# kngwyu/rogue-gym

Measured on AMD Instinct MI355X. Metric: env-steps/sec (whole node) at 65 536 envs, 32x16 mini-dungeon, higher is better.
Workload: dtype u8/u16 integer state, f32 observation; 1 GPU; config-mini.json 32x16, 65536 envs per GPU (65536 total), gray-image obs [N,1,16,32] f32, max_steps 1000, auto-reset; envs_per_gpu=65536, parallelism=env-sharded x1, no data-path collective

## Files before the change

### __graft_entry__.py

```python
import os
import subprocess
import sys

ROOT = os.path.dirname(os.path.abspath(__file__))
PKG = os.path.join(ROOT, "rogue-gym_amd")
for p in (ROOT, PKG):
    if p not in sys.path:
        sys.path.insert(0, p)


def source_id():
    import hashlib
    csrc = os.path.join(PKG, "csrc")
    files = sorted(os.path.join(csrc, f) for f in os.listdir(csrc) if f.endswith((".hip", ".cpp", ".h"))) + [os.path.join(ROOT, "include", "rogue_gym_hip.h")]
    h = hashlib.sha256()
    for f in files:
        h.update(os.path.basename(f).encode() + b"\0")
        h.update(open(f, "rb").read())
    return h.hexdigest()[:16]


def library_id(so):
    if not os.path.exists(so):
        return None
    blob = open(so, "rb").read()
    i = blob.find(b"RGBUILDID:")
    return blob[i + 10:i + 26].decode("ascii", "replace") if i >= 0 else None


def build():
    csrc = os.path.join(PKG, "csrc")
    so = os.path.join(PKG, "librogue_gym_hip.so")
    hipcc = "hipcc" if subprocess.call(["which", "hipcc"], stdout=subprocess.DEVNULL) == 0 else "/opt/rocm/bin/hipcc"
    sid = source_id()
    dev_so = os.path.join(PKG, "variants", "librogue_gym_hip_dev.so")
    nov_so = os.path.join(PKG, "librogue_gym_novelty.so")
    if library_id(so) != sid or library_id(dev_so) != sid or library_id(nov_so) != sid:
        have_hipcc = subprocess.call(["which", hipcc], stdout=subprocess.DEVNULL, stderr=subprocess.DEVNULL) == 0 or os.path.exists(hipcc)
        if have_hipcc:
            bdir = os.path.join(PKG, "build")
            os.makedirs(bdir, exist_ok=True)
            os.makedirs(os.path.dirname(dev_so), exist_ok=True)
            flags = ["--offload-arch=gfx950", "-std=c++17", "-fPIC", "-Wall", "-Wno-unused-function", '-DRG_BUILD_ID="%s"' % sid]
            objs, dev_objs, jobs = [], [], []
            for src, opt, has_knobs in (("rg_kernels.hip", "-O3", True), ("rg_regen_lanes.hip", "-O3", True), ("rg_obs.hip", "-Os", True), ("rg_crop_typed.hip", "-Os", False), ("rg_pixels.hip", "-Os", False), ("rg_action_mask.hip", "-Os", False), ("rg_path.hip", "-O3", False), ("rg_route.hip", "-O3", False), ("rg_episode.hip", "-O3", False), ("rg_monsters.hip", "-O3", False), ("rg_objects.hip", "-O3", False), ("rg_state_io.hip", "-O3", False), ("rg_api.cpp", "-O2", True), ("rg_config.cpp", "-O2", False),
                                        ("rg_items.cpp", "-O2", False)):
                obj = os.path.join(bdir, src.rsplit(".", 1)[0] + ".o")
                jobs.append(subprocess.Popen([hipcc] + flags + [opt, "-c", os.path.join(csrc, src), "-o", obj]))
                objs.append(obj)
                if has_knobs:
                    dobj = os.path.join(bdir, src.rsplit(".", 1)[0] + ".dev.o")
                    jobs.append(subprocess.Popen([hipcc] + flags + ["-DRG_DEV_KNOBS", opt, "-c", os.path.join(csrc, src), "-o", dobj]))
                    dev_objs.append(dobj)
                else:
                    dev_objs.append(obj)
            nov_obj = os.path.join(bdir, "rg_novelty.o")
            jobs.append(subprocess.Popen([hipcc] + flags + ["-O3", "-c", os.path.join(csrc, "rg_novelty.hip"), "-o", nov_obj]))
            if any(j.wait() != 0 for j in jobs):
                raise RuntimeError("hipcc failed")
            subprocess.check_call([hipcc, "--offload-arch=gfx950", "-shared", nov_obj, "-o", nov_so])
            link_nov = ["-L" + PKG, "-lrogue_gym_novelty"]
            subprocess.check_call([hipcc, "--offload-arch=gfx950", "-shared"] + objs + link_nov + ["-Wl,-rpath,$ORIGIN", "-o", so])
            subprocess.check_call([hipcc, "--offload-arch=gfx950", "-shared"] + dev_objs + link_nov + ["-Wl,-rpath,$ORIGIN/..", "-o", dev_so])
        elif not os.path.exists(so):
            raise RuntimeError("hipcc not found and librogue_gym_hip.so is not prebuilt")
        else:
            print("warning: hipcc not found; the prebuilt librogue_gym_hip.so (build id %s) does not match the sources (%s)" % (library_id(so), sid), file=sys.stderr)
    from oracle import pyoracle
    pyoracle.build()
    import rogue_gym
    from rogue_gym_python import _rogue_gym
    _rogue_gym.load_library()


def smoke():
    import json
    import numpy as np
    build()
    sys.path.insert(0, os.path.join(ROOT, "tests"))
    from parity_util import ACTION_KEYS, lockstep
    with open(os.path.join(ROOT, "tests", "golden", "reference_goldens.json")) as f:
        cfg = json.load(f)["configs"]["mini"]
    rng = np.random.RandomState(0)
    n, steps = 256, 64
    keys = [ACTION_KEYS[rng.randint(0, 11, n)] for _ in range(steps)]
    hip, _ = lockstep(cfg, list(range(n)), keys, max_steps=40, check_every=8, internal_every=32)
    obs = hip.obs(0, 0, False)
    assert obs.shape == (n, 1, 16, 32)
    print("smoke ok: %d envs x %d steps bit-exact vs oracle" % (n, steps))


if __name__ == "__main__":
    build()
    if len(sys.argv) > 1 and sys.argv[1] == "smoke":
# ... 2 lines not shown
```

### rogue-gym_amd/csrc/rg_api.cpp

```cpp
#include <hip/hip_runtime.h>
#include <dlfcn.h>

#include <algorithm>
#include <cstdio>
#include <cstdlib>
#include <cstring>
#include <mutex>
#include <random>
#include <string>
#include <vector>

#include "../../include/rogue_gym_hip.h"
#include "rg_state.h"
#include "rg_state_io.h"
#include "rg_readers_host.h"
#include "rg_pixels.h"

extern "C" {
typedef struct ncclComm *ncclComm_t;
typedef struct { char internal[128]; } ncclUniqueId;
typedef int ncclResult_t;
typedef int ncclDataType_t;
}
static const ncclResult_t ncclSuccess = 0;
static const ncclDataType_t ncclUint8 = 1;

extern "C" {
void rgk_build(const RgState *S, const RgConfig *c, hipStream_t st);
int rgk_step(const RgState *S, const RgState *SP_dev, const RgConfig *c, const uint8_t *keys, int use_spares, int parity, hipStream_t st, hipEvent_t ev0, hipEvent_t ev1);
void rgk_probe_clock(unsigned long long *out, int spin, hipStream_t st);
void rgk_regen(const RgState *SP, const RgConfig *c, int bulk, int spares, const uint32_t *mark, uint32_t target, uint32_t *err_any, hipStream_t st, hipEvent_t ev0, hipEvent_t ev1);
void rgk_regen_gate(const uint32_t *mark, uint32_t target, uint32_t *err_any, hipStream_t st);
void rgk_export(const RgState *S, uint32_t *err_any, void *o_screen, void *o_hist, void *o_status, void *o_flags, uint32_t *o_err, hipStream_t st);
int rgk_regen_lanes_supported(const RgConfig *c, int maze_cap);
int rgk_step_bound_capable(const RgConfig *c);
int rgk_regen_lanes(const RgState *SP, const RgConfig *c, uint32_t *q, int32_t *list, int bulk, int waves, int slots, hipStream_t st, hipEvent_t ev0, hipEvent_t ev1);
void rgk_debug_descend(const RgState *S, const RgConfig *c, hipStream_t st);
void rgk_render(const RgState *S, const RgConfig *c, hipStream_t st);
void rgk_encode(const uint8_t *screen, const uint8_t *hist, const int32_t *status, uint32_t *flags, uint32_t *err_any, int n, int hw, size_t rs, size_t rst,
                int symbols, int planes_sym, uint32_t sflag, int with_hist, int kind, float *out, const int32_t *ext, hipStream_t st);
void rgk_pack(const RgState *S, int with_hist, uint8_t *out, hipStream_t st);
void rgk_scatter_rows(const void *src, void *dst, const int32_t *ext, int n, int row_bytes, hipStream_t st);
void rgk_gather_keys(const uint8_t *keys, const int32_t *ext, uint8_t *dst, int n, hipStream_t st);
int rgk_obs(const RgState *S, const RgConfig *c, uint32_t sflag, int with_hist, int kind, float *out, uint32_t *err_any, int planes_sym, int bound, hipStream_t st, hipEvent_t ev0, hipEvent_t ev1);
int rgk_redraw(const RgState *S, const RgConfig *c, hipStream_t st);
int rgk_obs_tail_capable(const RgState *S, const RgConfig *c);
int rgk_step_tail_capable(const RgConfig *c);
int rgk_step_enc_helpers(int n, int want);
void rgk_obs_resid(const RgState *S, const RgConfig *c, float *out, hipStream_t st, hipEvent_t ev0, hipEvent_t ev1);
int rgk_obs_typed(const RgState *S, const RgConfig *c, int kind, int dtype, uint32_t sflag, int with_hist, int planes_sym, void *out, uint32_t *err_any, hipStream_t st, hipEvent_t ev0,
                  hipEvent_t ev1);
int rgk_crop_typed(const RgState *S, const RgConfig *c, int kind, int dtype, int ry, int rx, uint32_t sflag, int with_hist, int planes_sym, void *out, int32_t *centers,
                   uint32_t *err_any, hipStream_t st, hipEvent_t ev0, hipEvent_t ev1);
int rgk_pixels(const RgState *S, const RgConfig *c, const uint8_t *tiles, int th, int channels, int ry, int rx, uint8_t *out, int32_t *centers, hipStream_t st, hipEvent_t ev0,
               hipEvent_t ev1);
void rgk_action_mask(const RgState *S, const RgConfig *c, const uint8_t *keys, int n_keys, uint8_t *mask, uint8_t *sample, uint64_t seed, uint64_t draw, hipStream_t st,
                     hipEvent_t ev0, hipEvent_t ev1);
void rgk_path(const RgState *S, const RgConfig *c, uint32_t goals, const int32_t *gcell, uint16_t *field, int32_t *dist, uint8_t *key, hipStream_t st);
void rgk_route(const RgState *S, const RgConfig *c, uint32_t goals, uint32_t fallback, uint32_t mode, const int32_t *gcell, int32_t *dist, uint8_t *key, uint8_t *tier,
               hipStream_t st);
void rgk_episode(const RgState *S, const RgConfig *c, const RgEpisode *A, int slots, const int32_t *ids, const uint8_t *mask, int cut, int record, uint32_t serial,
                 hipStream_t st);
void rgk_novelty(const RgState *S, const RgConfig *c, const RgNovelty *A, int slots, const int32_t *ids, const uint8_t *mask, int cut, hipStream_t st);
void rgk_monsters(const RgState *S, const RgConfig *c, uint32_t mode, int cap, int16_t *table, int32_t *threat, hipStream_t st);
void rgk_objects(const RgState *S, const RgConfig *c, uint32_t kinds, uint32_t mode, int cap, int16_t *table, int32_t *count, hipStream_t st);
void rgk_state_save(const RgState *S, const RgIoLayout *L, const uint64_t *desc, const uint32_t *guard, const int32_t *ids, int k, uint8_t *out, hipStream_t st);
void rgk_state_load(const RgState *S, const RgIoLayout *L, const uint64_t *desc, const uint32_t *guard, const int32_t *ids, int k, const uint8_t *recs, uint32_t rec_bytes, uint8_t *ok,
                    uint8_t *mark, hipStream_t st);
void rgk_state_stairs(const RgState *S, const RgIoLayout *L, uint8_t *mark, hipStream_t st);
void rgk_reset_compact(const uint8_t *mask, int n, int32_t *list, uint32_t *cnt, hipStream_t st);
void rgk_build_list(const RgState *S, const RgConfig *c, const int32_t *list, const uint32_t *cnt, uint8_t *mark, hipStream_t st);
}

#define RG_ENC_DELAY_TICKS 2500u
#define RG_TIMED_KERNELS 5
struct rg_handle {
    RgParsed parsed;
    RgConfig cfg;
    RgState S;
    RgState SP;
    bool spares = false;
    uint32_t *lane_q = nullptr; int32_t *lane_list = nullptr;
    hipStream_t side3 = nullptr;
    hipStream_t side2 = nullptr;
    int lane_flip = 0;
    uint64_t lane_last = 0;
    uint8_t *pin_keys = nullptr;
    uint32_t *pin_err = nullptr;
    bool lane_regen = false;
    uint64_t step_count = 0;
    hipStream_t side = nullptr;
    int regen_idle_after = -1;
    int regen_bulk = 0;
    int device = 0;
    hipStream_t stream = nullptr;
    std::vector<void *> allocs;
    uint32_t *d_err = nullptr;
    uint8_t *d_keys = nullptr;
    bool render_pending = false;
    float *bound_out = nullptr; int bound_kind = 0; bool bound_valid = false;
    int32_t *obs_list_mem = nullptr; uint32_t *obs_cnt_mem = nullptr; float *gray_lut_mem = nullptr;
    bool tail_enc = false, tail_enc_off = false;
    int enc_helpers = 0;
    int bound_steps = 0;
    int stair_gen = 0;
    float *obs_scratch = nullptr;
    size_t obs_scratch_cap = 0;
    std::vector<uint64_t> seed_lo, seed_hi;
    std::vector<uint8_t> reseed;
    std::vector<uint64_t> range_lo, range_span;
    unsigned long long *d_probe = nullptr;
    std::vector<rg_handle *> sub;
    std::vector<int> g_of, l_of;
    int32_t *d_ext = nullptr;
    std::vector<int32_t> ext;
    uint8_t *d_keys_sub = nullptr;
    int planes_sym = 0;
    bool screens_stale = true;
    bool mixed = false;
    std::vector<size_t> ragged_off;
    size_t stat_rows = 0;
    RgState *d_SP = nullptr;
    ncclComm_t comm = nullptr;
    int comm_rank = 0, comm_world = 1;
    std::string err;
    bool timing = false;
    std::vector<hipEvent_t> ev[RG_TIMED_KERNELS];
    size_t ev_used[RG_TIMED_KERNELS] = {0, 0, 0, 0, 0};
    uint64_t timing_seq[RG_TIMED_KERNELS] = {0, 0, 0, 0, 0};
    uint64_t timing_stride = 1;
    uint64_t state_fp = 0;
    uint64_t *io_desc = nullptr;
    uint32_t *io_guard = nullptr;
    uint32_t io_words = 0;
    int32_t *io_ids = nullptr; size_t io_ids_cap = 0;
// ... 426 lines not shown
    return upload_seeds(h, (size_t)n);
}

int rg_reset(rg_t *h) {
    HIPCHK(h, hipSetDevice(h->device));
    if (!h->sub.empty()) {
        for (rg_handle *sh : h->sub) SUBCHK(h, sh, rg_reset(sh));
        h->screens_stale = true;
        return assemble_small(h);
    }
    h->S.stair_gen = h->stair_gen++;
    { TimedLaunch t(h, 3); rgk_build(&h->S, &h->cfg, h->stream); }
    HIPCHK(h, hipGetLastError());
    h->render_pending = true;
    h->bound_valid = false;
    return 0;
}

static int obs_common(rg_t *h, uint32_t status_flag, int with_hist, int kind, float *out_dev);
int rg_step(rg_t *h, const uint8_t *keys, int keys_on_device) { return rg_step_prefix(h, keys, h->S.n, keys_on_device); }
int rg_step_obs_gray(rg_t *h, const uint8_t *keys, int keys_on_device, uint32_t status_flag, int with_hist, float *out_dev) {
    const bool enc = h->tail_enc && !h->tail_enc_off && h->sub.empty() && (status_flag & 0x1ffu) == 0 && !with_hist && !h->bound_out && out_dev && rgk_obs_tail_capable(&h->S, &h->cfg);
    if (enc) {
        h->S.enc_out = out_dev;
        h->S.enc_helpers = h->enc_helpers;
    }
    const int rc = rg_step_prefix(h, keys, h->S.n, keys_on_device);
    h->S.enc_out = nullptr;
    h->S.enc_helpers = 0;
    if (rc) return 1;
    if (!enc) return obs_common(h, status_flag, with_hist, 0, out_dev);
    {
        TimedLaunch t(h, 2, true);
        rgk_obs_resid(&h->S, &h->cfg, out_dev, h->stream, t.start_ev(), t.stop_ev());
    }
    HIPCHK(h, hipGetLastError());
    h->render_pending = false;
    h->bound_valid = false;
    h->bound_steps = 0;
    return 0;
}

int rg_step_prefix(rg_t *h, const uint8_t *keys, int n_keys, int keys_on_device) {
    HIPCHK(h, hipSetDevice(h->device));
    if (n_keys < 0) { h->err = "rg_step_prefix: negative key count"; return 1; }
    if (n_keys > h->S.n) n_keys = h->S.n;
    if (!h->sub.empty()) {
        const uint8_t *dkeys = keys;
        if (!keys_on_device) {
            if (!h->d_keys && !dev_alloc(h, &h->d_keys, (size_t)h->S.n)) return 1;
            HIPCHK(h, hipMemcpyAsync(h->d_keys, keys, (size_t)n_keys, hipMemcpyHostToDevice, h->stream));
            dkeys = h->d_keys;
        }
        for (rg_handle *sh : h->sub) {
            int m = 0;
            while (m < sh->S.n && sh->ext[m] < n_keys) m++;
            if (m) rgk_gather_keys(dkeys, sh->d_ext, sh->d_keys_sub, m, h->stream);
            SUBCHK(h, sh, rg_step_prefix(sh, sh->d_keys_sub, m, 1));
        }
        HIPCHK(h, hipGetLastError());
        h->screens_stale = true;
        return assemble_small(h);
    }
    if (flush_render(h)) return 1;
    const uint8_t *dk = keys;
    if (!keys_on_device) {
        HIPCHK(h, hipMemcpyAsync(h->d_keys, keys, (size_t)n_keys, hipMemcpyHostToDevice, h->stream));
// ... 47 lines not shown
    }
    uint32_t err = 0;
    HIPCHK(h, hipMemcpyAsync(&err, h->d_err, 4, hipMemcpyDeviceToHost, h->stream));
    HIPCHK(h, hipStreamSynchronize(h->stream));
    if (h->side) { HIPCHK(h, hipStreamSynchronize(h->side)); HIPCHK(h, hipStreamSynchronize(h->side2)); HIPCHK(h, hipStreamSynchronize(h->side3)); }
    if (err) {
        HIPCHK(h, hipMemsetAsync(h->d_err, 0, 4, h->stream));
        if (err & RG_FLAG_ERR_INTERNAL) h->err = "internal capacity guard of the HIP stepper tripped (please report the config), or rg_reset_envs was given a device-side env id out of range";
        else if (err & RG_FLAG_ERR_STATE) h->err = "state record refused: it does not fit this env (magic / version / config fingerprint / geometry), the env is unchanged";
        else if (err & RG_FLAG_ERR_KEY) h->err = "Invalid input (key is not in the ai keymap)";
        else if (err & RG_FLAG_ERR_DEAD) h->err = "Ignored input (action while the player is dead)";
        else h->err = "Invalid tile in symbol image (symbol >= symbols - 1)";
        return 1;
    }
    return 0;
}

static int flush_mirrors(rg_handle *h) { return h->sub.empty() ? flush_render(h) : assemble_screens(h); }
int rg_screen(rg_t *h, uint8_t **dev) { if (refuse_mixed(h, "rg_screen")) return 1; HIPCHK(h, hipSetDevice(h->device)); if (flush_mirrors(h)) return 1; *dev = h->S.screen; return 0; }
int rg_hist(rg_t *h, uint8_t **dev) { if (refuse_mixed(h, "rg_hist")) return 1; HIPCHK(h, hipSetDevice(h->device)); if (flush_mirrors(h)) return 1; *dev = h->S.hist; return 0; }
int rg_status(rg_t *h, int32_t **dev) { *dev = h->S.status; return 0; }
int rg_flags(rg_t *h, uint32_t **dev) { HIPCHK(h, hipSetDevice(h->device)); if (flush_mirrors(h)) return 1; *dev = h->S.flags; return 0; }
int rg_reward(rg_t *h, float **dev) { *dev = h->S.reward; return 0; }
int rg_done(rg_t *h, uint8_t **dev) { *dev = h->S.done; return 0; }
int rg_set_stair_reward(rg_t *h, float bonus) {
    if (!(bonus == bonus) || bonus < 0.f) { h->err = "rg_set_stair_reward: the bonus must be a number >= 0"; return 1; }
    h->S.stair_reward = bonus;
    for (rg_handle *sh : h->sub) sh->S.stair_reward = bonus;
    return 0;
}

int rg_tail_encode(rg_t *h, int on) {
    h->tail_enc_off = on == 0;
    for (rg_handle *sh : h->sub) sh->tail_enc_off = on == 0;
    return 0;
}

int rg_obs_channels(const rg_t *h, int symbol, uint32_t status_flag, int with_hist) {
    return (symbol ? h->planes_sym : 1) + __builtin_popcount(status_flag & 0x1ffu) + (with_hist ? 1 : 0);
}

static int symbols_check(rg_t *h, const std::string &w, const rg_handle *sh) {
    if (sh->cfg.symbols <= h->planes_sym) return 0;
    h->err = w + "symbol image: a config of the batch has more symbols (" + std::to_string(sh->cfg.symbols) + ") than env 0's (" + std::to_string(h->planes_sym) +
             "), which sets the channel count (python/src/lib.rs:281-285)";
    return 1;
}
static int obs_common(rg_t *h, uint32_t status_flag, int with_hist, int kind, float *out_dev) {
    if (refuse_mixed(h, kind ? "rg_obs_symbol" : "rg_obs_gray")) return 1;
    HIPCHK(h, hipSetDevice(h->device));
    if (!h->sub.empty()) {
        for (rg_handle *sh : h->sub) {
            if (kind && symbols_check(h, "", sh)) return 1;
            SUBCHK(h, sh, obs_common(sh, status_flag, with_hist, kind, out_dev));
        }
        return 0;
    }
    {
        TimedLaunch t(h, 2, true);
        const bool bound = h->bound_out && out_dev == h->bound_out && kind == h->bound_kind && (status_flag & 0x1ffu) == 0 && !with_hist;
        if (rgk_obs(&h->S, &h->cfg, status_flag & 0x1ffu, with_hist ? 1 : 0, kind, out_dev, h->d_err, h->planes_sym, bound && h->S.obs_list && h->bound_valid && h->bound_steps == 1, h->stream, t.start_ev(), t.stop_ev())) {
            HIPCHK(h, hipGetLastError());
            h->render_pending = false;
            h->bound_valid = bound;
            h->bound_steps = 0;
            return 0;
        }
// ... 1313 lines not shown
```

### rogue-gym_amd/csrc/rg_obs.hip

```cpp
#include <cstdlib>
#include "rg_device.h"

#define RENDER_THREADS 256
__device__ __forceinline__ bool in_same_room(const RgState &S, const RgConfig &c, int e, int ax, int ay, int bx, int by) {
    int id = room_id_of(c, ax, ay);
    if (id < 0 || room_id_of(c, bx, by) != id) return false;
    uint8_t meta = S.room_meta[id * S.n + e];
    if ((meta & RM_KIND_MASK) == RK_EMPTY) return true;
    int x0, y0, x1, y1;
    unpack_rect(S.room_rect[id * S.n + e], x0, y0, x1, y1);
    bool ina = ax >= x0 && ax < x1 && ay >= y0 && ay < y1, inb = bx >= x0 && bx < x1 && by >= y0 && by < y1;
    return ina == inb;
}

__global__ void __launch_bounds__(RENDER_THREADS) k_render(RgState S, RgConfig c) {
    __shared__ uint8_t s_scr[RG_MAX_W * RG_MAX_H];
    const int tid = threadIdx.x, W = c.width, H = c.height, HW = W * H, n = S.n;
    const int nrooms = c.room_num_x * c.room_num_y;
    for (int e = blockIdx.x; e < n; e += gridDim.x) {
        const uint32_t fl = S.flags[e];
        if (!(fl & RG_FLAG_REDRAW)) continue;
        const uint16_t *cell = S.cell + (size_t)e * HW;
        const bool upd_hist = !(fl & RG_FLAG_HIST_STALE);
        uint8_t *hist = S.hist + (size_t)e * HW;
// ... 89 lines not shown
    for (size_t g = (size_t)blockIdx.x * blockDim.x + threadIdx.x; g < total; g += (size_t)gridDim.x * blockDim.x) {
        int e = (int)(g / q), i = (int)(g - (size_t)e * q);
        uint32_t s4 = reinterpret_cast<const uint32_t *>(screen + (size_t)e * rs)[i];
        uint32_t a = tile_to_sym(s4 & 0xff), b = tile_to_sym((s4 >> 8) & 0xff), cc = tile_to_sym((s4 >> 16) & 0xff), d = tile_to_sym(s4 >> 24);
        if (a >= symbol_max || b >= symbol_max || cc >= symbol_max || d >= symbol_max) {
            if (flags) atomicOr(&flags[e], RG_FLAG_ERR_TILE);
            atomicOr(err_any, RG_FLAG_ERR_TILE);
        }
        float4 *o = reinterpret_cast<float4 *>(out + (size_t)(ext ? ext[e] : e) * nplanes * hw) + i;
        for (uint32_t ch = 0; ch < (uint32_t)planes_sym; ch++) {
            float4 v;
            v.x = a == ch ? 1.f : 0.f; v.y = b == ch ? 1.f : 0.f; v.z = cc == ch ? 1.f : 0.f; v.w = d == ch ? 1.f : 0.f;
            if (ch >= symbol_max) v.x = v.y = v.z = v.w = 0.f;
            o[(size_t)ch * q] = v;
        }
        int p = planes_sym;
        for (int bb = 0; bb < 9; bb++)
            if (sflag & (1u << bb)) {
                float f = (float)status[(size_t)e * rst + kStatusIdx[bb]];
                float4 sv; sv.x = sv.y = sv.z = sv.w = f;
                o[(size_t)p * q] = sv;
                p++;
            }
        if (with_hist) {
            uint32_t h4 = reinterpret_cast<const uint32_t *>(hist + (size_t)e * rs)[i];
            float4 hv;
            hv.x = (h4 & 0xff) ? 1.f : 0.f; hv.y = (h4 & 0xff00) ? 1.f : 0.f; hv.z = (h4 & 0xff0000) ? 1.f : 0.f; hv.w = (h4 >> 24) ? 1.f : 0.f;
            o[(size_t)p * q] = hv;
        }
    }
}

#define OBS_THREADS 256
__device__ __forceinline__ void store_obs(float4 *p, float4 v) {
    typedef float f4v __attribute__((ext_vector_type(4)));
    f4v nv = {v.x, v.y, v.z, v.w};
#ifdef RG_EXP_OBS_PLAIN_STORES
    *reinterpret_cast<f4v *>(p) = nv;
#else
    __builtin_nontemporal_store(nv, reinterpret_cast<f4v *>(p));
#endif
}
struct ObsTabs { uint32_t w[RG_OBS_REC_WORDS(RG_OBS_MAX_ROOMS)]; };
#define OBS_ENV_BYTES(hw) ((((size_t)(hw) + sizeof(ObsTabs)) + 15) & ~(size_t)15)

__device__ __forceinline__ void draw_cells8(uint4 v, int i, int W, int HW, uint32_t g[2], uint32_t hb[2]) {
    const uint32_t q[4] = {v.x, v.y, v.z, v.w};
    g[0] = g[1] = hb[0] = hb[1] = 0;
#pragma unroll
    for (int t = 0; t < 8; t++) {
        uint32_t cw = (q[t >> 1] >> ((t & 1) * 16)) & 0xffff;
        int idx = i * 8 + t;
        bool inner = idx >= W && idx < HW - W;
        uint32_t gl = ' ';
        if (inner && (cw & C_VISIBLE)) gl = glyph_of(cw);
        if (inner && (cw & (C_VISIBLE | C_DRAWN))) gl = ((cw & C_GOLD) ? (uint32_t)'*' : gl) | 0x80u;
        g[t >> 2] |= gl << ((t & 3) * 8);
        hb[t >> 2] |= ((cw & C_VISITED) ? 1u : 0u) << ((t & 3) * 8);
    }
}
__device__ __forceinline__ bool monster_shown(const RgConfig &c, const ObsTabs *tb, int nrooms, int px, int py, int x, int y) {
    int dx = px - x, dy = py - y;
    bool show = dx * dx + dy * dy <= 2;
    if (!show) {
        int id = room_id_of(c, px, py);
        if (id >= 0 && room_id_of(c, x, y) == id) {
            if ((reinterpret_cast<const uint8_t *>(&tb->w[2 * nrooms + 1])[id] & RM_KIND_MASK) == RK_EMPTY) show = true;
            else {
                int x0, y0, x1, y1;
                unpack_rect(tb->w[nrooms + 1 + id], x0, y0, x1, y1);
                bool ina = px >= x0 && px < x1 && py >= y0 && py < y1, inb = x >= x0 && x < x1 && y >= y0 && y < y1;
                show = ina == inb;
            }
        }
    }
    return show;
}

template <int KIND, bool GROUPS, bool BOUND = false>
__global__ void __launch_bounds__(OBS_THREADS) k_obs(RgState S, RgConfig c, uint32_t sflag, int with_hist, float *__restrict__ out,
                                                    uint32_t *__restrict__ err_any, int tpe, int epb, int planes_sym, int hi_prio) {
    if (hi_prio) __builtin_amdgcn_s_setprio(3);
    extern __shared__ __align__(16) uint8_t smem[];
    float *lutf = reinterpret_cast<float *>(smem);
    uint8_t *luts = smem + 512;
    uint8_t *mtile = smem + 512 + 128;
    uint8_t *envs = smem + 512 + 128 + 64;
    const int tid = threadIdx.x, W = c.width, H = c.height, HW = W * H, Q8 = HW >> 3;
    const int32_t *list = BOUND ? S.obs_list + (size_t)S.obs_par * S.n : nullptr;
    const int n = BOUND ? (int)S.obs_cnt[S.obs_par] : S.n;
    const int nrooms = c.room_num_x * c.room_num_y;
    const int symbols = c.symbols;
    for (int g = tid; g < 128; g += blockDim.x) {
        uint32_t sy = tile_to_sym((uint32_t)g);
        luts[g] = (uint8_t)sy;
        lutf[g] = (float)(uint8_t)sy / (float)(uint8_t)symbols;
    }
    for (int g = tid; g < RG_MAX_ENEMY_KINDS + 6; g += blockDim.x) mtile[g] = c.mon[g].tile;
    const int le = tid / tpe, lt = tid - le * tpe;
    const int base_planes = KIND ? (GROUPS ? planes_sym : symbols) : 1;
    const int nplanes = base_planes + __popc(sflag) + (with_hist ? 1 : 0);
    uint8_t *scr = envs + (size_t)le * OBS_ENV_BYTES(HW);
    ObsTabs *tb = reinterpret_cast<ObsTabs *>(scr + HW);
    struct Pre { uint4 v0; uint32_t rec; };
    const int rec_words = RG_OBS_REC_WORDS(nrooms);
    const uint32_t *rec_all = S.obs_rec;
    const int stride = gridDim.x * epb;
    const int Q4 = HW >> 2;
    const bool one_wave = blockDim.x == WAVE;
    const bool fast_ok = (epb == 1 || one_wave) && Q4 <= 4 * tpe && sflag == 0 && !with_hist;
// ... 125 lines not shown
        if (redraw && lt == 0 && (scr[py * W + px] & 0x80u)) scr[py * W + px] = (uint8_t)(0x80u | '@');
        lds_barrier();
        if (with_hist) __syncthreads();
        if (staged) {
            uint32_t *m4 = reinterpret_cast<uint32_t *>(S.screen + (size_t)e * HW);
            const uint32_t *scr4 = reinterpret_cast<const uint32_t *>(scr);
            const uint32_t *hist4 = reinterpret_cast<const uint32_t *>(S.hist + (size_t)e * HW);
            const int xe = GROUPS ? __builtin_amdgcn_readfirstlane(S.ext[e]) : e;
            float4 *o = reinterpret_cast<float4 *>(out + (size_t)xe * nplanes * HW);
            float stf[9];
            int nst = 0;
            for (int b = 0; b < 9; b++)
                if (sflag & (1u << b)) stf[nst++] = (float)S.status[(size_t)e * 10 + kStatusIdx[b]];
            bool bad = false;
            for (int q = lt; q < Q4; q += tpe) {
                const uint32_t g = scr4[q] & 0x7f7f7f7fu;
                if (redraw) m4[q] = g;
                emit(o, q, g, stf, nst, hist4, bad);
            }
            if (KIND == 1 && bad) { atomicOr(&S.flags[e], RG_FLAG_ERR_TILE); atomicOr(err_any, RG_FLAG_ERR_TILE); }
            const uint32_t seen = BOUND ? RG_FLAG_SCR_CHANGED : 0u;
            if (redraw && lt == 0) {
                const uint32_t clr = seen | RG_FLAG_REDRAW | RG_FLAG_HIST_STALE | RG_FLAG_HIST_LAG | ((fl & RG_FLAG_HIST_STALE) ? 0u : RG_FLAG_HIST_DIRTY);
                const uint32_t set = (fl & RG_FLAG_HIST_STALE) ? RG_FLAG_HIST_LAG : 0u;
                if (KIND == 1) {
                    atomicAnd(&S.flags[e], ~clr);
                    if (set) atomicOr(&S.flags[e], set);
                } else S.flags[e] = (fl & ~clr) | set;
            } else if (BOUND && !redraw && lt == 0) atomicAnd(&S.flags[e], ~RG_FLAG_SCR_CHANGED);
        }
    }
}

#define RG_OBS_REDRAW_ENV() \
    lds_barrier();                                                                                                             \
    if (lane < rec_words) tb.w[lane] = t_rec;                                                                                                                            \
                           \
    const bool upd_hist = !(fle & RG_FLAG_HIST_STALE) && (fle & RG_FLAG_HIST_DIRTY);                                                                                     \
    if (lane < Q8) {                                                                                                                                                     \
        uint32_t g[2], hb[2];                                                                                                                                            \
        draw_cells8(v, lane, W, HW, g, hb);                                                                                                                              \
        reinterpret_cast<uint2 *>(scr)[lane] = make_uint2(g[0], g[1]);                                                                                                   \
        if (upd_hist) reinterpret_cast<uint2 *>(S.hist + (size_t)e * HW)[lane] = make_uint2(hb[0], hb[1]);                                                               \
    }                                                                                                                                                                    \
    lds_barrier();                                                                                                                                                       \
                                                                      \
    const uint32_t ppos = tb.w[nrooms];                                                                                                                                  \
    const int px = POS_X(ppos), py = POS_Y(ppos);                                                                                                                        \
    if (lane < nrooms) {                                                                                                                                                 \
        const uint32_t mw = tb.w[lane];                                                                                                                                  \
        if ((mw >> 24) & MF_ALIVE) {                                                                                                                                     \
            const int x = POS_X(mw), y = POS_Y(mw);                                                                                                                      \
            const uint32_t under = scr[y * W + x];                                                                                                                       \
            if (monster_shown(c, &tb, nrooms, px, py, x, y) && (under & 0x80u) && under != (0x80u | '*')) scr[y * W + x] = (uint8_t)(0x80u | mtile[(mw >> 16) & 0xff]);  \
        }                                                                                                                                                                \
    }                                                                                                                                                                    \
    lds_barrier();                                                                                                                                                       \
    if (lane == 0 && (scr[py * W + px] & 0x80u)) scr[py * W + px] = (uint8_t)(0x80u | '@');                                                                              \
    lds_barrier();                                                                                                                                                       \
    uint32_t *m4 = reinterpret_cast<uint32_t *>(S.screen + (size_t)e * HW);                                                                                              \
    float4 *oe = reinterpret_cast<float4 *>(out) + (size_t)e * Q4;                                                                                                       \
    for (int q = lane; q < Q4; q += WAVE) {                                                                                                                              \
        const uint32_t g = reinterpret_cast<const uint32_t *>(scr)[q] & 0x7f7f7f7fu;                                                                                     \
        m4[q] = g;                                                                                                                                                       \
        store_obs(&oe[q], gray4(g));                                                                                                                                     \
    }                                                                                                                                                                    \
    if (lane == 0)                                                                    \
        S.flags[e] = (fle & ~(RG_FLAG_REDRAW | RG_FLAG_HIST_STALE | RG_FLAG_HIST_LAG | ((fle & RG_FLAG_HIST_STALE) ? 0u : RG_FLAG_HIST_DIRTY))) |                        \
                     ((fle & RG_FLAG_HIST_STALE) ? RG_FLAG_HIST_LAG : 0u);

#ifndef OBS_RUN
#define OBS_RUN 4
#endif
#ifndef OBS_STREAM_WAVES
#define OBS_STREAM_WAVES 16384
#endif
__global__ void __launch_bounds__(WAVE) k_obs_stream(RgState S, RgConfig c, float *__restrict__ out, int hi_prio) {
    if (hi_prio) __builtin_amdgcn_s_setprio(3);
    __shared__ float lutf[128];
    __shared__ uint8_t mtile[RG_MAX_ENEMY_KINDS + 6];
    __shared__ __align__(16) uint8_t scr[512];
    __shared__ ObsTabs tb;
    const int lane = threadIdx.x, W = c.width, HW = W * c.height, Q4 = HW >> 2, Q8 = HW >> 3, n = S.n;
    const int nrooms = c.room_num_x * c.room_num_y, rec_words = RG_OBS_REC_WORDS(nrooms);
    for (int g = lane; g < 128; g += WAVE) lutf[g] = (float)(uint8_t)tile_to_sym((uint32_t)g) / (float)(uint8_t)c.symbols;
    for (int g = lane; g < RG_MAX_ENEMY_KINDS + 6; g += WAVE) mtile[g] = c.mon[g].tile;
    lds_barrier();
    auto gray4 = [&](uint32_t w) {
        w &= 0x7f7f7f7fu;
        float4 v; v.x = lutf[w & 0xff]; v.y = lutf[(w >> 8) & 0xff]; v.z = lutf[(w >> 16) & 0xff]; v.w = lutf[w >> 24];
        return v;
    };
    struct Run { uint32_t fl, w0[OBS_RUN], w1[OBS_RUN]; };
    auto load_run = [&](int r, Run &R) {
        const int base = r * OBS_RUN, cnt = n - base;
        R.fl = lane < cnt && lane < OBS_RUN ? S.flags[base + lane] : 0u;
        const uint32_t *m = reinterpret_cast<const uint32_t *>(S.screen) + (size_t)base * Q4;
#pragma unroll
        for (int i = 0; i < OBS_RUN; i++) {
            R.w0[i] = i < cnt && lane < Q4 ? m[i * Q4 + lane] : 0u;
            R.w1[i] = i < cnt && lane + WAVE < Q4 ? m[i * Q4 + lane + WAVE] : 0u;
        }
// ... 515 lines not shown
```

### rogue-gym_amd/rogue_gym_python/_rogue_gym.py

```python
import ctypes as C
import operator
import weakref
import json
import os

import numpy as np

_HERE = os.path.dirname(os.path.abspath(__file__))
_SO = os.environ.get("ROGUE_GYM_HIP_LIB") or os.path.join(os.path.dirname(_HERE), "librogue_gym_hip.so")

RG_FLAG_TERMINAL = 0x1
RG_FLAG_DEAD = 0x2
RG_FLAG_MSG_SHIFT = 8
RG_FLAG_MSG_MASK = 0x7F00
RG_FLAG_ERR_MASK = 0x00FF0000

STATUS_KEYS = ("dungeon_level", "gold", "hp_current", "hp_max", "str_current", "str_max", "defense", "player_level", "exp", "hunger")


class RgDebugState(C.Structure):
    _fields_ = [
        ("px", C.c_int32), ("py", C.c_int32), ("dungeon_level", C.c_int32), ("hp", C.c_int32), ("hp_max", C.c_int32),
        ("player_level", C.c_int32), ("n_monsters", C.c_int32), ("n_gold", C.c_int32),
        ("exp", C.c_uint32), ("food_left", C.c_uint32), ("quiet", C.c_uint32), ("pack_gold", C.c_uint32), ("steps", C.c_uint32),
# ... 389 lines not shown

def _route_args(goal, fallback=None, secrets=False, known=False, with_cells=False):
    def word(name, what):
        if not isinstance(name, str) or name not in ROUTE_GOALS:
            raise ValueError("%s must be one of %s, got %r" % (what, ", ".join(repr(g) for g in ROUTE_GOALS), name))
        return ROUTE_GOALS[name]
    goals = 4 if (goal is None and with_cells) else word(goal, "goal") | (4 if with_cells else 0)
    fb = 0 if fallback is None else word(fallback, "fallback")
    if ((goals | fb) & 8) and not known:
        raise ValueError("the goal 'frontier' needs known=True: the frontier is of the player's own map")
    return goals, fb, (ROUTE_SECRETS if secrets else 0) | (ROUTE_KNOWN if known else 0)


class _Handle:

    def __init__(self, configs, max_steps, auto_reset, device=None):
        L = load_library()
        self.L = L
        self.device = _default_device() if device is None else device
        n = len(configs)
        arr = (C.c_char_p * n)()
        for i, cfg in enumerate(configs):
            arr[i] = None if cfg is None else cfg.encode("utf-8")
        h = C.c_void_p()
        rc = L.rg_create(arr, n, int(max_steps), self.device, int(auto_reset), C.byref(h))
        if rc:
            msg = L.rg_last_error(None).decode()
            if msg.startswith("Failed to parse config"):
                raise RuntimeError(msg)
            raise RuntimeError("Error in rogue-gym: " + msg)
        self.h = h
        if os.environ.get("ROGUE_GYM_HIP_NO_TAIL_ENCODE", "0") not in ("", "0") and hasattr(L, "rg_tail_encode"):
            L.rg_tail_encode(h, 0)
        hh, ww, ss, nn = C.c_int(), C.c_int(), C.c_int(), C.c_int()
        L.rg_dims(h, C.byref(hh), C.byref(ww), C.byref(ss), C.byref(nn))
        self.height, self.width, self.symbols, self.n = hh.value, ww.value, ss.value, nn.value
        self.env_symbols = np.empty(self.n, np.int32)
        L.rg_env_symbols(h, self.env_symbols.ctypes.data)
        self.uniform_symbols = bool((self.env_symbols == self.symbols).all())
        self.env_heights, self.env_widths = np.empty(self.n, np.int32), np.empty(self.n, np.int32)
        L.rg_env_dims(h, self.env_heights.ctypes.data, self.env_widths.ctypes.data)
        self.mixed_sizes = bool((self.env_heights != self.height).any() or (self.env_widths != self.width).any())
        self.pool = _PinnedPool(L)
        self.dev_pool = _DevPool(L, self.device)
        self.lazy = {}
        self.epoch = 0
        self.fast_step = True
        self._mask_dev = None

    def check(self, rc):
        if rc:
            raise RuntimeError("Error in rogue-gym: " + self.L.rg_last_error(self.h).decode())

    def close(self):
        if getattr(self, "h", None):
            for ref in list(self.lazy.values()):
                b = ref()
                if b is not None:
                    b._materialise()
            if self._mask_dev is not None:
                self.L.rg_dev_free(self.device, C.c_void_p(self._mask_dev[0]))
                self._mask_dev = None
            self.L.rg_destroy(self.h)
            self.h = None
            self.pool.close()
            self.dev_pool.close()
# ... 594 lines not shown
```

Before: 869.1 million env-steps/s.

## Replace residual obs pass with per-line fixup kernel compacting dirty rows per group

Adds a new fixup kernel used by default in the tail-encode observation path, replacing the old residual pass. Each wave covers a group of 16 envs, builds a compacted list of dirty screen lines from enc_rows via prefix sums, converts only those lines to float, and batches full redraws per wave. The goal is to touch only the lines that changed and balance work across lanes rather than scanning whole envs. It adds a separate shared library plus env knobs for bounds experiments, and correctness depends on enc_rows being accurate.

Result: no change. 877.3 million env-steps/s, median of 6 (+0.9%).

```diff
diff --git a/__graft_entry__.py b/__graft_entry__.py
--- a/__graft_entry__.py
+++ b/__graft_entry__.py
@@ -35,7 +35,8 @@
     sid = source_id()
     dev_so = os.path.join(PKG, "variants", "librogue_gym_hip_dev.so")
     nov_so = os.path.join(PKG, "librogue_gym_novelty.so")
-    if library_id(so) != sid or library_id(dev_so) != sid or library_id(nov_so) != sid:
+    fix_so = os.path.join(PKG, "librogue_gym_fixup.so")
+    if library_id(so) != sid or library_id(dev_so) != sid or library_id(nov_so) != sid or library_id(fix_so) != sid:
         have_hipcc = subprocess.call(["which", hipcc], stdout=subprocess.DEVNULL, stderr=subprocess.DEVNULL) == 0 or os.path.exists(hipcc)
         if have_hipcc:
             bdir = os.path.join(PKG, "build")
@@ -56,10 +57,13 @@
                     dev_objs.append(obj)
             nov_obj = os.path.join(bdir, "rg_novelty.o")
             jobs.append(subprocess.Popen([hipcc] + flags + ["-O3", "-c", os.path.join(csrc, "rg_novelty.hip"), "-o", nov_obj]))
+            fix_obj = os.path.join(bdir, "rg_obs_fix.o")
+            jobs.append(subprocess.Popen([hipcc] + flags + ["-Os", "-c", os.path.join(csrc, "rg_obs_fix.hip"), "-o", fix_obj]))
             if any(j.wait() != 0 for j in jobs):
                 raise RuntimeError("hipcc failed")
             subprocess.check_call([hipcc, "--offload-arch=gfx950", "-shared", nov_obj, "-o", nov_so])
-            link_nov = ["-L" + PKG, "-lrogue_gym_novelty"]
+            subprocess.check_call([hipcc, "--offload-arch=gfx950", "-shared", fix_obj, "-o", fix_so])
+            link_nov = ["-L" + PKG, "-lrogue_gym_novelty", "-lrogue_gym_fixup"]
             subprocess.check_call([hipcc, "--offload-arch=gfx950", "-shared"] + objs + link_nov + ["-Wl,-rpath,$ORIGIN", "-o", so])
             subprocess.check_call([hipcc, "--offload-arch=gfx950", "-shared"] + dev_objs + link_nov + ["-Wl,-rpath,$ORIGIN/..", "-o", dev_so])
         elif not os.path.exists(so):
diff --git a/rogue-gym_amd/csrc/rg_api.cpp b/rogue-gym_amd/csrc/rg_api.cpp
--- a/rogue-gym_amd/csrc/rg_api.cpp
+++ b/rogue-gym_amd/csrc/rg_api.cpp
@@ -48,6 +48,8 @@
 int rgk_step_tail_capable(const RgConfig *c);
 int rgk_step_enc_helpers(int n, int want);
 void rgk_obs_resid(const RgState *S, const RgConfig *c, float *out, hipStream_t st, hipEvent_t ev0, hipEvent_t ev1);
+void rgk_obs_fix(const RgState *S, const RgConfig *c, float *out, hipStream_t st, hipEvent_t ev0, hipEvent_t ev1);
+void rgk_obs_fix_bound(const RgState *S, const RgConfig *c, float *out, hipStream_t st, hipEvent_t ev0, hipEvent_t ev1, uint32_t bound);
 int rgk_obs_typed(const RgState *S, const RgConfig *c, int kind, int dtype, uint32_t sflag, int with_hist, int planes_sym, void *out, uint32_t *err_any, hipStream_t st, hipEvent_t ev0,
                   hipEvent_t ev1);
 int rgk_crop_typed(const RgState *S, const RgConfig *c, int kind, int dtype, int ry, int rx, uint32_t sflag, int with_hist, int planes_sym, void *out, int32_t *centers,
@@ -100,7 +102,7 @@
     bool render_pending = false;
     float *bound_out = nullptr; int bound_kind = 0; bool bound_valid = false;
     int32_t *obs_list_mem = nullptr; uint32_t *obs_cnt_mem = nullptr; float *gray_lut_mem = nullptr;
-    bool tail_enc = false, tail_enc_off = false;
+    bool tail_enc = false, tail_enc_off = false, fix_resid = false;
     int enc_helpers = 0;
     int bound_steps = 0;
     int stair_gen = 0;
@@ -593,7 +595,13 @@
     if (!enc) return obs_common(h, status_flag, with_hist, 0, out_dev);
     {
         TimedLaunch t(h, 2, true);
-        rgk_obs_resid(&h->S, &h->cfg, out_dev, h->stream, t.start_ev(), t.stop_ev());
+        bool old_pass = h->fix_resid;
+        uint32_t bound = 0;
+        if (const char *ev = RG_DEV_ENV("RG_OBS_RESID_BLOCKS")) old_pass = old_pass || atoi(ev) > 0;
+        if (const char *ev = RG_DEV_ENV("RG_OBS_FIX_BOUND")) bound = !strcmp(ev, "null") ? 1u : !strcmp(ev, "lines") ? 2u : !strcmp(ev, "redraws") ? 3u : 0u;
+        if (old_pass) rgk_obs_resid(&h->S, &h->cfg, out_dev, h->stream, t.start_ev(), t.stop_ev());
+        else if (bound) rgk_obs_fix_bound(&h->S, &h->cfg, out_dev, h->stream, t.start_ev(), t.stop_ev(), bound);
+        else rgk_obs_fix(&h->S, &h->cfg, out_dev, h->stream, t.start_ev(), t.stop_ev());
     }
     HIPCHK(h, hipGetLastError());
     h->render_pending = false;
@@ -707,7 +715,8 @@
 
 int rg_tail_encode(rg_t *h, int on) {
     h->tail_enc_off = on == 0;
-    for (rg_handle *sh : h->sub) sh->tail_enc_off = on == 0;
+    h->fix_resid = on == 2;
+    for (rg_handle *sh : h->sub) { sh->tail_enc_off = on == 0; sh->fix_resid = on == 2; }
     return 0;
 }
 
diff --git a/rogue-gym_amd/csrc/rg_obs.hip b/rogue-gym_amd/csrc/rg_obs.hip
--- a/rogue-gym_amd/csrc/rg_obs.hip
+++ b/rogue-gym_amd/csrc/rg_obs.hip
@@ -145,50 +145,7 @@
 }
 
 #define OBS_THREADS 256
-__device__ __forceinline__ void store_obs(float4 *p, float4 v) {
-    typedef float f4v __attribute__((ext_vector_type(4)));
-    f4v nv = {v.x, v.y, v.z, v.w};
-#ifdef RG_EXP_OBS_PLAIN_STORES
-    *reinterpret_cast<f4v *>(p) = nv;
-#else
-    __builtin_nontemporal_store(nv, reinterpret_cast<f4v *>(p));
-#endif
-}
-struct ObsTabs { uint32_t w[RG_OBS_REC_WORDS(RG_OBS_MAX_ROOMS)]; };
-#define OBS_ENV_BYTES(hw) ((((size_t)(hw) + sizeof(ObsTabs)) + 15) & ~(size_t)15)
-
-__device__ __forceinline__ void draw_cells8(uint4 v, int i, int W, int HW, uint32_t g[2], uint32_t hb[2]) {
-    const uint32_t q[4] = {v.x, v.y, v.z, v.w};
-    g[0] = g[1] = hb[0] = hb[1] = 0;
-#pragma unroll
-    for (int t = 0; t < 8; t++) {
-        uint32_t cw = (q[t >> 1] >> ((t & 1) * 16)) & 0xffff;
-        int idx = i * 8 + t;
-        bool inner = idx >= W && idx < HW - W;
-        uint32_t gl = ' ';
-        if (inner && (cw & C_VISIBLE)) gl = glyph_of(cw);
-        if (inner && (cw & (C_VISIBLE | C_DRAWN))) gl = ((cw & C_GOLD) ? (uint32_t)'*' : gl) | 0x80u;
-        g[t >> 2] |= gl << ((t & 3) * 8);
-        hb[t >> 2] |= ((cw & C_VISITED) ? 1u : 0u) << ((t & 3) * 8);
-    }
-}
-__device__ __forceinline__ bool monster_shown(const RgConfig &c, const ObsTabs *tb, int nrooms, int px, int py, int x, int y) {
-    int dx = px - x, dy = py - y;
-    bool show = dx * dx + dy * dy <= 2;
-    if (!show) {
-        int id = room_id_of(c, px, py);
-        if (id >= 0 && room_id_of(c, x, y) == id) {
-            if ((reinterpret_cast<const uint8_t *>(&tb->w[2 * nrooms + 1])[id] & RM_KIND_MASK) == RK_EMPTY) show = true;
-            else {
-                int x0, y0, x1, y1;
-                unpack_rect(tb->w[nrooms + 1 + id], x0, y0, x1, y1);
-                bool ina = px >= x0 && px < x1 && py >= y0 && py < y1, inb = x >= x0 && x < x1 && y >= y0 && y < y1;
-                show = ina == inb;
-            }
-        }
-    }
-    return show;
-}
+#include "rg_obs_draw.h"
 
 template <int KIND, bool GROUPS, bool BOUND = false>
 __global__ void __launch_bounds__(OBS_THREADS) k_obs(RgState S, RgConfig c, uint32_t sflag, int with_hist, float *__restrict__ out,
@@ -380,42 +337,6 @@
     }
 }
 
-#define RG_OBS_REDRAW_ENV() \
-    lds_barrier();                                                                                                             \
-    if (lane < rec_words) tb.w[lane] = t_rec;                                                                                                                            \
-                           \
-    const bool upd_hist = !(fle & RG_FLAG_HIST_STALE) && (fle & RG_FLAG_HIST_DIRTY);                                                                                     \
-    if (lane < Q8) {                                                                                                                                                     \
-        uint32_t g[2], hb[2];                                                                                                                                            \
-        draw_cells8(v, lane, W, HW, g, hb);                                                                                                                              \
-        reinterpret_cast<uint2 *>(scr)[lane] = make_uint2(g[0], g[1]);                                                                                                   \
-        if (upd_hist) reinterpret_cast<uint2 *>(S.hist + (size_t)e * HW)[lane] = make_uint2(hb[0], hb[1]);                                                               \
-    }                                                                                                                                                                    \
-    lds_barrier();                                                                                                                                                       \
-                                                                      \
-    const uint32_t ppos = tb.w[nrooms];                                                                                                                                  \
-    const int px = POS_X(ppos), py = POS_Y(ppos);                                                                                                                        \
-    if (lane < nrooms) {                                                                                                                                                 \
-        const uint32_t mw = tb.w[lane];                                                                                                                                  \
-        if ((mw >> 24) & MF_ALIVE) {                                                                                                                                     \
-            const int x = POS_X(mw), y = POS_Y(mw);                                                                                                                      \
-            const uint32_t under = scr[y * W + x];                                                                                                                       \
-            if (monster_shown(c, &tb, nrooms, px, py, x, y) && (under & 0x80u) && under != (0x80u | '*')) scr[y * W + x] = (uint8_t)(0x80u | mtile[(mw >> 16) & 0xff]);  \
-        }                                                                                                                                                                \
-    }                                                                                                                                                                    \
-    lds_barrier();                                                                                                                                                       \
-    if (lane == 0 && (scr[py * W + px] & 0x80u)) scr[py * W + px] = (uint8_t)(0x80u | '@');                                                                              \
-    lds_barrier();                                                                                                                                                       \
-    uint32_t *m4 = reinterpret_cast<uint32_t *>(S.screen + (size_t)e * HW);                                                                                              \
-    float4 *oe = reinterpret_cast<float4 *>(out) + (size_t)e * Q4;                                                                                                       \
-    for (int q = lane; q < Q4; q += WAVE) {                                                                                                                              \
-        const uint32_t g = reinterpret_cast<const uint32_t *>(scr)[q] & 0x7f7f7f7fu;                                                                                     \
-        m4[q] = g;                                                                                                                                                       \
-        store_obs(&oe[q], gray4(g));                                                                                                                                     \
-    }                                                                                                                                                                    \
-    if (lane == 0)                                                                    \
-        S.flags[e] = (fle & ~(RG_FLAG_REDRAW | RG_FLAG_HIST_STALE | RG_FLAG_HIST_LAG | ((fle & RG_FLAG_HIST_STALE) ? 0u : RG_FLAG_HIST_DIRTY))) |                        \
-                     ((fle & RG_FLAG_HIST_STALE) ? RG_FLAG_HIST_LAG : 0u);
 
 #ifndef OBS_RUN
 #define OBS_RUN 4
diff --git a/rogue-gym_amd/csrc/rg_obs_draw.h b/rogue-gym_amd/csrc/rg_obs_draw.h
--- /dev/null
+++ b/rogue-gym_amd/csrc/rg_obs_draw.h
@@ -0,0 +1,84 @@
+#pragma once
+#include "rg_device.h"
+
+__device__ __forceinline__ void store_obs(float4 *p, float4 v) {
+    typedef float f4v __attribute__((ext_vector_type(4)));
+    f4v nv = {v.x, v.y, v.z, v.w};
+#ifdef RG_EXP_OBS_PLAIN_STORES
+    *reinterpret_cast<f4v *>(p) = nv;
+#else
+    __builtin_nontemporal_store(nv, reinterpret_cast<f4v *>(p));
+#endif
+}
+struct ObsTabs { uint32_t w[RG_OBS_REC_WORDS(RG_OBS_MAX_ROOMS)]; };
+#define OBS_ENV_BYTES(hw) ((((size_t)(hw) + sizeof(ObsTabs)) + 15) & ~(size_t)15)
+
+__device__ __forceinline__ void draw_cells8(uint4 v, int i, int W, int HW, uint32_t g[2], uint32_t hb[2]) {
+    const uint32_t q[4] = {v.x, v.y, v.z, v.w};
+    g[0] = g[1] = hb[0] = hb[1] = 0;
+#pragma unroll
+    for (int t = 0; t < 8; t++) {
+        uint32_t cw = (q[t >> 1] >> ((t & 1) * 16)) & 0xffff;
+        int idx = i * 8 + t;
+        bool inner = idx >= W && idx < HW - W;
+        uint32_t gl = ' ';
+        if (inner && (cw & C_VISIBLE)) gl = glyph_of(cw);
+        if (inner && (cw & (C_VISIBLE | C_DRAWN))) gl = ((cw & C_GOLD) ? (uint32_t)'*' : gl) | 0x80u;
+        g[t >> 2] |= gl << ((t & 3) * 8);
+        hb[t >> 2] |= ((cw & C_VISITED) ? 1u : 0u) << ((t & 3) * 8);
+    }
+}
+__device__ __forceinline__ bool monster_shown(const RgConfig &c, const ObsTabs *tb, int nrooms, int px, int py, int x, int y) {
+    int dx = px - x, dy = py - y;
+    bool show = dx * dx + dy * dy <= 2;
+    if (!show) {
+        int id = room_id_of(c, px, py);
+        if (id >= 0 && room_id_of(c, x, y) == id) {
+            if ((reinterpret_cast<const uint8_t *>(&tb->w[2 * nrooms + 1])[id] & RM_KIND_MASK) == RK_EMPTY) show = true;
+            else {
+                int x0, y0, x1, y1;
+                unpack_rect(tb->w[nrooms + 1 + id], x0, y0, x1, y1);
+                bool ina = px >= x0 && px < x1 && py >= y0 && py < y1, inb = x >= x0 && x < x1 && y >= y0 && y < y1;
+                show = ina == inb;
+            }
+        }
+    }
+    return show;
+}
+
+#define RG_OBS_REDRAW_ENV() \
+    lds_barrier();                                                                                                             \
+    if (lane < rec_words) tb.w[lane] = t_rec;                                                                                                                            \
+                           \
+    const bool upd_hist = !(fle & RG_FLAG_HIST_STALE) && (fle & RG_FLAG_HIST_DIRTY);                                                                                     \
+    if (lane < Q8) {                                                                                                                                                     \
+        uint32_t g[2], hb[2];                                                                                                                                            \
+        draw_cells8(v, lane, W, HW, g, hb);                                                                                                                              \
+        reinterpret_cast<uint2 *>(scr)[lane] = make_uint2(g[0], g[1]);                                                                                                   \
+        if (upd_hist) reinterpret_cast<uint2 *>(S.hist + (size_t)e * HW)[lane] = make_uint2(hb[0], hb[1]);                                                               \
+    }                                                                                                                                                                    \
+    lds_barrier();                                                                                                                                                       \
+                                                                      \
+    const uint32_t ppos = tb.w[nrooms];                                                                                                                                  \
+    const int px = POS_X(ppos), py = POS_Y(ppos);                                                                                                                        \
+    if (lane < nrooms) {                                                                                                                                                 \
+        const uint32_t mw = tb.w[lane];                                                                                                                                  \
+        if ((mw >> 24) & MF_ALIVE) {                                                                                                                                     \
+            const int x = POS_X(mw), y = POS_Y(mw);                                                                                                                      \
+            const uint32_t under = scr[y * W + x];                                                                                                                       \
+            if (monster_shown(c, &tb, nrooms, px, py, x, y) && (under & 0x80u) && under != (0x80u | '*')) scr[y * W + x] = (uint8_t)(0x80u | mtile[(mw >> 16) & 0xff]);  \
+        }                                                                                                                                                                \
+    }                                                                                                                                                                    \
+    lds_barrier();                                                                                                                                                       \
+    if (lane == 0 && (scr[py * W + px] & 0x80u)) scr[py * W + px] = (uint8_t)(0x80u | '@');                                                                              \
+    lds_barrier();                                                                                                                                                       \
+    uint32_t *m4 = reinterpret_cast<uint32_t *>(S.screen + (size_t)e * HW);                                                                                              \
+    float4 *oe = reinterpret_cast<float4 *>(out) + (size_t)e * Q4;                                                                                                       \
+    for (int q = lane; q < Q4; q += WAVE) {                                                                                                                              \
+        const uint32_t g = reinterpret_cast<const uint32_t *>(scr)[q] & 0x7f7f7f7fu;                                                                                     \
+        m4[q] = g;                                                                                                                                                       \
+        store_obs(&oe[q], gray4(g));                                                                                                                                     \
+    }                                                                                                                                                                    \
+    if (lane == 0)                                                                    \
+        S.flags[e] = (fle & ~(RG_FLAG_REDRAW | RG_FLAG_HIST_STALE | RG_FLAG_HIST_LAG | ((fle & RG_FLAG_HIST_STALE) ? 0u : RG_FLAG_HIST_DIRTY))) |                        \
+                     ((fle & RG_FLAG_HIST_STALE) ? RG_FLAG_HIST_LAG : 0u);
diff --git a/rogue-gym_amd/csrc/rg_obs_fix.h b/rogue-gym_amd/csrc/rg_obs_fix.h
--- /dev/null
+++ b/rogue-gym_amd/csrc/rg_obs_fix.h
@@ -0,0 +1,17 @@
+#pragma once
+#include <hip/hip_runtime.h>
+#include "rg_state.h"
+
+#define RG_FIX_BOUND_NONE 0u
+#define RG_FIX_BOUND_NULL 1u
+#define RG_FIX_BOUND_LINES 2u
+#define RG_FIX_BOUND_REDRAWS 3u
+
+extern "C" {
+int rgk_obs_fix_group(void);
+int rgk_obs_fix_split(int n);
+int rgk_obs_fix_blocks(int n);
+void rgk_obs_fix(const RgState *S, const RgConfig *c, float *out, hipStream_t st, hipEvent_t ev0, hipEvent_t ev1);
+void rgk_obs_fix_bound(const RgState *S, const RgConfig *c, float *out, hipStream_t st, hipEvent_t ev0, hipEvent_t ev1, uint32_t bound);
+const char *rgk_obs_fix_build_id(void);
+}
diff --git a/rogue-gym_amd/csrc/rg_obs_fix.hip b/rogue-gym_amd/csrc/rg_obs_fix.hip
--- /dev/null
+++ b/rogue-gym_amd/csrc/rg_obs_fix.hip
@@ -0,0 +1,137 @@
+#include "rg_device.h"
+#include "rg_obs_draw.h"
+#include "rg_obs_fix.h"
+#include "rg_obs_fix_pack.h"
+
+#ifndef OBS_FIX_GROUP
+#define OBS_FIX_GROUP 16
+#endif
+#ifndef OBS_FIX_REDRAWS
+#define OBS_FIX_REDRAWS 4
+#endif
+#ifndef OBS_FIX_SPLIT_MAX
+#define OBS_FIX_SPLIT_MAX 4
+#endif
+#ifndef OBS_FIX_WAVES
+#define OBS_FIX_WAVES 4096
+#endif
+#ifndef OBS_FIX_DEPTH
+#define OBS_FIX_DEPTH 4
+#endif
+static_assert(OBS_FIX_GROUP == 16 || OBS_FIX_GROUP == 32 || OBS_FIX_GROUP == 64, "a group is a power-of-two part of a wave");
+
+__global__ void __launch_bounds__(WAVE) k_obs_fix(RgState S, RgConfig c, float *__restrict__ out, uint32_t bound, uint32_t split) {
+    __shared__ float lutf[128];
+    __shared__ uint8_t mtile[RG_MAX_ENEMY_KINDS + 6];
+    __shared__ __align__(16) uint8_t scr[512];
+    __shared__ ObsTabs tb;
+    __shared__ uint16_t items[OBS_FIX_GROUP * RG_FIX_LINES];
+    const int lane = threadIdx.x, W = c.width, HW = W * c.height, Q4 = HW >> 2, Q8 = HW >> 3, n = S.n;
+    const int nrooms = c.room_num_x * c.room_num_y, rec_words = RG_OBS_REC_WORDS(nrooms);
+    const uint32_t part = blockIdx.x % split;
+    const int base = (int)(blockIdx.x / split) * OBS_FIX_GROUP;
+    const bool in = lane < OBS_FIX_GROUP && base + lane < n;
+    uint32_t fl = in ? S.flags[base + lane] : 0u;
+    uint32_t rows = in ? (uint32_t)S.enc_rows[base + lane] : 0u;
+    if ((uint32_t)lane % split != part) fl = rows = 0u;
+    lutf[lane] = S.gray_lut[lane];
+    lutf[lane + WAVE] = S.gray_lut[lane + WAVE];
+    for (int g = lane; g < RG_MAX_ENEMY_KINDS + 6; g += WAVE) mtile[g] = c.mon[g].tile;
+    auto gray4 = [&](uint32_t w) {
+        w &= 0x7f7f7f7fu;
+        float4 v; v.x = lutf[w & 0xff]; v.y = lutf[(w >> 8) & 0xff]; v.z = lutf[(w >> 16) & 0xff]; v.w = lutf[w >> 24];
+        return v;
+    };
+    if (bound == RG_FIX_BOUND_LINES) fl &= ~RG_FLAG_REDRAW;
+    const bool redraw = (fl & RG_FLAG_REDRAW) != 0u;
+    uint64_t rmask = __ballot(redraw);
+    const uint32_t cnt = rg_fix_count(redraw, rows);
+    uint32_t incl = cnt;
+#pragma unroll
+    for (int off = 1; off < OBS_FIX_GROUP; off <<= 1) {
+        const uint32_t up = __shfl_up(incl, off);
+        if (lane >= off) incl += up;
+    }
+    uint32_t total = __builtin_amdgcn_readlane(incl, OBS_FIX_GROUP - 1);
+    if (bound == RG_FIX_BOUND_REDRAWS) total = 0u;
+    if (bound == RG_FIX_BOUND_NULL) return;
+    if (!(rmask | total)) return;
+    uint4 tv[OBS_FIX_REDRAWS];
+    uint32_t trec[OBS_FIX_REDRAWS];
+    int ri[OBS_FIX_REDRAWS];
+    auto load_redraws = [&]() {
+#pragma unroll
+        for (int r = 0; r < OBS_FIX_REDRAWS; r++) {
+            tv[r] = make_uint4(0, 0, 0, 0);
+            trec[r] = 0u;
+            ri[r] = -1;
+            if (rmask) {
+                ri[r] = __builtin_ctzll(rmask);
+                rmask &= rmask - 1;
+                const int e = base + ri[r];
+                if (lane < Q8) tv[r] = reinterpret_cast<const uint4 *>(S.cell + (size_t)e * HW)[lane];
+                if (lane < rec_words) trec[r] = S.obs_rec[(size_t)e * rec_words + lane];
+            }
+        }
+    };
+    load_redraws();
+    if (cnt && total) rg_fix_fill(items, lane, incl - cnt, rows);
+    lds_barrier();
+    const uint32_t *m = reinterpret_cast<const uint32_t *>(S.screen) + (size_t)base * Q4;
+    float4 *o = reinterpret_cast<float4 *>(out) + (size_t)base * Q4;
+    const uint32_t nslots = rg_fix_slots(total);
+    for (uint32_t s0 = 0; s0 < nslots; s0 += OBS_FIX_DEPTH) {
+        int at[OBS_FIX_DEPTH];
+        uint32_t w[OBS_FIX_DEPTH];
+#pragma unroll
+        for (int d = 0; d < OBS_FIX_DEPTH; d++) {
+            const uint32_t j = rg_fix_slot_item(s0 + d, lane);
+            at[d] = -1;
+            w[d] = 0u;
+            if (j < total) {
+                at[d] = rg_fix_word_index(items[j], lane, Q4);
+                w[d] = m[at[d]];
+            }
+        }
+#pragma unroll
+        for (int d = 0; d < OBS_FIX_DEPTH; d++)
+            if (at[d] >= 0) store_obs(&o[at[d]], gray4(w[d]));
+    }
+    for (;;) {
+#pragma unroll
+        for (int r = 0; r < OBS_FIX_REDRAWS; r++) {
+            if (ri[r] < 0) continue;
+            const int e = base + ri[r];
+            const uint32_t fle = __builtin_amdgcn_readlane(fl, ri[r]);
+            const uint4 v = tv[r];
+            const uint32_t t_rec = trec[r];
+            RG_OBS_REDRAW_ENV();
+        }
+        if (!rmask) break;
+        load_redraws();
+    }
+}
+
+#ifndef RG_BUILD_ID
+#define RG_BUILD_ID "unstamped"
+#endif
+extern "C" {
+const char *rgk_obs_fix_build_id(void) { static const char id[] = "RGBUILDID:" RG_BUILD_ID; return id + 10; }
+int rgk_obs_fix_group(void) { return OBS_FIX_GROUP; }
+static int fix_groups(int n) {
+    const int groups = n > 0 ? (int)(((long long)n + OBS_FIX_GROUP - 1) / OBS_FIX_GROUP) : 0;
+    return groups < 1 ? 1 : groups;
+}
+int rgk_obs_fix_split(int n) {
+    int split = 1;
+    while (split < OBS_FIX_SPLIT_MAX && (long long)fix_groups(n) * split * 2 <= OBS_FIX_WAVES) split *= 2;
+    return split;
+}
+int rgk_obs_fix_blocks(int n) { return fix_groups(n) * rgk_obs_fix_split(n); }
+void rgk_obs_fix_bound(const RgState *S, const RgConfig *c, float *out, hipStream_t st, hipEvent_t ev0, hipEvent_t ev1, uint32_t bound) {
+    rg_launch(k_obs_fix, dim3(rgk_obs_fix_blocks(S->n)), dim3(WAVE), 0, st, ev0, ev1, *S, *c, out, bound, (uint32_t)rgk_obs_fix_split(S->n));
+}
+void rgk_obs_fix(const RgState *S, const RgConfig *c, float *out, hipStream_t st, hipEvent_t ev0, hipEvent_t ev1) {
+    rgk_obs_fix_bound(S, c, out, st, ev0, ev1, RG_FIX_BOUND_NONE);
+}
+}
diff --git a/rogue-gym_amd/csrc/rg_obs_fix_pack.h b/rogue-gym_amd/csrc/rg_obs_fix_pack.h
--- /dev/null
+++ b/rogue-gym_amd/csrc/rg_obs_fix_pack.h
@@ -0,0 +1,26 @@
+#pragma once
+#include <cstdint>
+
+#if defined(__HIPCC__) || defined(__CUDACC__)
+#define RG_FIX_HD __host__ __device__ __forceinline__
+#else
+#define RG_FIX_HD inline
+#endif
+
+#define RG_FIX_LINES 16
+#define RG_FIX_LINE_WORDS 8
+#define RG_FIX_SLOT_ITEMS 8
+#define RG_FIX_ITEM(env, line) ((uint16_t)(((env) << 4) | (line)))
+#define RG_FIX_ITEM_ENV(it) ((int)(it) >> 4)
+#define RG_FIX_ITEM_LINE(it) ((int)(it) & 15)
+
+RG_FIX_HD uint32_t rg_fix_count(int redraw, uint32_t mask) { return redraw ? 0u : (uint32_t)__builtin_popcount(mask & 0xffffu); }
+RG_FIX_HD uint32_t rg_fix_fill(uint16_t *items, int env, uint32_t first, uint32_t mask) {
+    uint32_t k = 0;
+    for (uint32_t m = mask & 0xffffu; m; m &= m - 1u) items[first + k++] = RG_FIX_ITEM(env, __builtin_ctz(m));
+    return k;
+}
+RG_FIX_HD uint32_t rg_fix_slots(uint32_t total) { return (total + RG_FIX_SLOT_ITEMS - 1u) / RG_FIX_SLOT_ITEMS; }
+RG_FIX_HD uint32_t rg_fix_slot_item(uint32_t slot, int lane) { return slot * RG_FIX_SLOT_ITEMS + ((uint32_t)lane >> 3); }
+RG_FIX_HD int rg_fix_slot_word(int lane) { return lane & (RG_FIX_LINE_WORDS - 1); }
+RG_FIX_HD int rg_fix_word_index(uint16_t item, int lane, int q4) { return RG_FIX_ITEM_ENV(item) * q4 + RG_FIX_ITEM_LINE(item) * RG_FIX_LINE_WORDS + rg_fix_slot_word(lane); }
diff --git a/rogue-gym_amd/rogue_gym_python/_rogue_gym.py b/rogue-gym_amd/rogue_gym_python/_rogue_gym.py
--- a/rogue-gym_amd/rogue_gym_python/_rogue_gym.py
+++ b/rogue-gym_amd/rogue_gym_python/_rogue_gym.py
@@ -445,6 +445,8 @@
         self.h = h
         if os.environ.get("ROGUE_GYM_HIP_NO_TAIL_ENCODE", "0") not in ("", "0") and hasattr(L, "rg_tail_encode"):
             L.rg_tail_encode(h, 0)
+        elif os.environ.get("ROGUE_GYM_HIP_FIXUP_RESID", "0") not in ("", "0") and hasattr(L, "rg_tail_encode"):
+            L.rg_tail_encode(h, 2)
         hh, ww, ss, nn = C.c_int(), C.c_int(), C.c_int(), C.c_int()
         L.rg_dims(h, C.byref(hh), C.byref(ww), C.byref(ss), C.byref(nn))
         self.height, self.width, self.symbols, self.n = hh.value, ww.value, ss.value, nn.value
```
